# zhihu/rucene

Hardware: NVIDIA H100
Metric: queries/sec (higher is better)
Workload: dtype u32/f32

## Files before the change

### rucene_b200/csrc/gpu/eval_shared.cuh

```cuda
#pragma once
#include "engine.hpp"
#include "unpack.cuh"

namespace rg {

constexpr int kEvalThreads = 256;
constexpr int kEvalWarps = kEvalThreads / 32;
constexpr int kNewcMax = 512;
constexpr int kMaxK = 1024;
constexpr uint32_t kNone = 0xffffffffu;
constexpr uint32_t kRunMin = 256;
constexpr uint32_t kRunFirst = 63;
constexpr uint32_t kSent = 0x7fc0dead;
constexpr uint32_t kExcl = 0x7fc0beef;

struct EmitShared {
    float topk[kMaxK];
    float newc[kNewcMax];
    uint32_t warp_c[kEvalWarps], warp_m[kEvalWarps];
    uint32_t newc_n;
    uint32_t topk_n;
    float theta_local;
    uint32_t theta_in;
    uint32_t run_slot, run_cap, run_cnt;
// ... 207 lines not shown
        }
    }
    __syncthreads();
    if (nc && !es.overflow) {
        uint32_t pos = es.write_base + es.warp_c[warp];
        const uint32_t lt = (1u << lane) - 1u;
#pragma unroll
        for (int s = 0; s < STEPS; s++) {
            if ((cmask[s] >> lane) & 1u) {
                p.cand_arena[pos + __popc(cmask[s] & lt)] = rg_hit{doc[s] + doc_base, score[s]};
                const uint32_t i = atomicAdd(&es.newc_n, 1u);
                if (DEEP) deep_count(reinterpret_cast<uint32_t*>(es.topk), dmap, score[s]);
                else if (i < (uint32_t)kNewcMax) es.newc[i] = score[s];
            }
            pos += __popc(cmask[s]);
        }
    }
    __syncthreads();
    if (warp == 0) {
        if (DEEP) theta_update_deep(es, p, item_idx, dmap);
        else theta_update(es, p.k, p.item_theta + item_idx);
    }
}

__device__ __forceinline__ uint32_t lower_bound_i32(const int32_t* __restrict__ a, uint32_t lo,
                                                    uint32_t hi, int32_t key) {
    while (lo < hi) {
        const uint32_t mid = (lo + hi) >> 1;
        if (__ldg(a + mid) < key) lo = mid + 1;
        else hi = mid;
    }
    return lo;
}
__device__ __forceinline__ uint32_t lower_bound_gallop(const int32_t* __restrict__ a, uint32_t hint,
                                                       uint32_t n, int32_t key) {
    uint32_t lo = hint, step = 1, hi = hint;
    while (hi < n && __ldg(a + hi) < key) {
        lo = hi + 1;
        hi += step;
        step <<= 1;
    }
    return lower_bound_i32(a, lo, min(hi, n), key);
}

struct TermCtx {
    const int32_t* blk_last;
    const BlockDesc* blk_desc;
    const float* cache;
    uint32_t nb;
    uint32_t cur;
    uint32_t next_cur;
    uint32_t tail_n;
    uint32_t tail_pos;
    uint32_t tail_next;
    int32_t tail_base;
    float w1;
};

static __device__ void decode_tail(const SegDev& seg, const TermDev& td, int32_t* docs, int32_t* freqs) {
    if (td.doc_freq == 1) {
        docs[0] = td.singleton_doc;
        freqs[0] = td.singleton_freq;
        return;
    }
    const uint8_t* p = seg.tails + td.tail_off;
    uint32_t pos = 0;
    int32_t acc = td.tail_base;
    for (uint32_t i = 0; i < td.tail_n; i++) {
        const uint32_t code = (uint32_t)read_vint(p, pos);
        acc += (int32_t)(code >> 1);
        docs[i] = acc;
        freqs[i] = (code & 1u) ? 1 : read_vint(p, pos);
    }
}

__device__ __forceinline__ bool is_live(const SegDev& seg, int doc) {
    if (!seg.live) return true;
    return (seg.live[doc >> 6] >> (doc & 63)) & 1ull;
}

constexpr int kOrWarps = 1;
constexpr int kOrThreads = kOrWarps * 32;
constexpr int kWw = 768;
constexpr int kNewcW = 64;

struct WTerm {
    const int32_t* blk_last;
    union {
        const BlockDesc* blk_desc;
        const uint32_t* col_bmax;
    };
    union {
        const float* cache;
        const uint32_t* col_bits;
    };
    uint32_t nb;
    uint32_t cur;
    uint32_t n;
    uint32_t pos;
    uint32_t term_id;
    float w1;
    uint32_t is_not;
    uint32_t is_col;
    union {
        const uint4* pre;
        unsigned long long* col_dbg;
    };
};

struct MsmCtx {
    uint8_t* cnt;
    uint32_t msm;
    float* mx;
};
template <bool NOT, bool MSM, bool DMAX, bool POS = false>
__device__ __forceinline__ void accumulate_posting(uint32_t* acc, int idx, float s, bool is_not, bool live,
                                                   float te, uint32_t& hot, uint32_t& my_matches,
                                                   const MsmCtx& mc) {
    if (POS) {
        acc[idx] = __float_as_uint(__fadd_rn(__uint_as_float(acc[idx]), s));
        return;
    }
    const uint32_t old = acc[idx];
    if (!NOT || !is_not) {
        const float sum = __fadd_rn(old == kSent ? 0.0f : __uint_as_float(old), s);
        acc[idx] = __float_as_uint(sum);
        if (DMAX) mc.mx[idx] = old == kSent ? s : fmaxf(mc.mx[idx], s);
        if (MSM) {
            const uint32_t c = (uint32_t)mc.cnt[idx] + 1u;
            mc.cnt[idx] = (uint8_t)c;
            if (c == mc.msm && live) my_matches++;
        } else if (old == kSent && live) {
            my_matches++;
        }
        if (DMAX || sum > te) hot |= 1u << (idx >> 5);
    } else if (old != kSent && old != kExcl) {
        acc[idx] = kExcl;
        if (live && (!MSM || mc.cnt[idx] >= mc.msm)) my_matches--;
    }
}

struct alignas(16) WarpShared {
    uint32_t acc[kWw];
    WTerm term[kMaxTerms];
    float newc[kNewcW];
};

struct WEmit {
    float* topk;
    bool mirror;
    uint32_t topk_n;
    float theta_local;
    uint32_t theta_in;
    uint32_t run_slot, run_cap, run_cnt;
    uint32_t matches;
    bool overflow;
};

__device__ __forceinline__ void wtheta_recompute(const WEmit& em, uint32_t k, int lane, float& theta, int& argmin) {
    float m = INFINITY;
    int mi = 0;
    for (uint32_t j = lane; j < k; j += 32) {
        const float v = em.topk[j];
        if (v < m) {
            m = v;
            mi = (int)j;
        }
// ... 266 lines not shown
```

### rucene_b200/csrc/gpu/query_kernels.cu

```cuda
#include <algorithm>

#include "eval_shared.cuh"

namespace rg {


template <bool LIVE, bool EDGE, bool POS>
__device__ __forceinline__ void column_window(uint32_t* acc, const float* __restrict__ col, bool every_doc,
                                              const SegDev& seg, int win0, int wlen, int first_in, float te, int lane,
                                              uint32_t& hot, uint32_t& my_matches) {
    if (POS && !EDGE && wlen == kWw) {
#pragma unroll
        for (int h = 0; h < kWw / 128; h += 3) {
            float4 v[3];
#pragma unroll
            for (int j = 0; j < 3; j++) v[j] = __ldg(reinterpret_cast<const float4*>(col + win0 + lane * 4 + (h + j) * 128));
#pragma unroll
            for (int j = 0; j < 3; j++) {
                float4* a = reinterpret_cast<float4*>(acc + lane * 4 + (h + j) * 128);
                const float4 o = *a;
                *a = make_float4(__fadd_rn(o.x, v[j].x), __fadd_rn(o.y, v[j].y), __fadd_rn(o.z, v[j].z), __fadd_rn(o.w, v[j].w));
            }
        }
        return;
    }
#pragma unroll 2
    for (int i = lane * 4; i < wlen; i += 128) {
        const int d0 = win0 + i;
        const float4 v = __ldg(reinterpret_cast<const float4*>(col + d0));
        float sv[4] = {v.x, v.y, v.z, v.w};
        const uint4 o4 = *reinterpret_cast<const uint4*>(acc + i);
        uint32_t o[4] = {o4.x, o4.y, o4.z, o4.w};
        bool any_hot = false;
        if (POS) {
#pragma unroll
            for (int q = 0; q < 4; q++) {
                if (EDGE) sv[q] = (i + q >= first_in && i + q < wlen) ? sv[q] : 0.0f;
                o[q] = __float_as_uint(__fadd_rn(__uint_as_float(o[q]), sv[q]));
            }
        } else {
            uint32_t live4 = 0xfu;
            if (LIVE && seg.live) live4 = (uint32_t)(seg.live[d0 >> 6] >> (d0 & 63)) & 0xfu;
#pragma unroll
            for (int q = 0; q < 4; q++) {
                bool present = every_doc || sv[q] != 0.0f;
                if (EDGE) present = present && i + q >= first_in && i + q < wlen;
                const bool fresh = o[q] == kSent;
                const float sum = __fadd_rn(fresh ? 0.0f : __uint_as_float(o[q]), sv[q]);
                o[q] = present ? __float_as_uint(sum) : o[q];
                my_matches += (fresh && present && (!LIVE || ((live4 >> q) & 1u))) ? 1u : 0u;
                any_hot |= present && sum > te;
            }
        }
        *reinterpret_cast<uint4*>(acc + i) = make_uint4(o[0], o[1], o[2], o[3]);
        if (!POS) hot |= any_hot ? 1u << (i >> 5) : 0u;
    }
}

__device__ __forceinline__ uint32_t min1(uint32_t x) {
    uint32_t r;
    asm("min.u32 %0, %1, 1;" : "=r"(r) : "r"(x));
    return r;
}
template <bool LIVE>
__device__ __forceinline__ void count_and_max(const uint4 o, int g, int lane, const uint64_t* __restrict__ live, int win0,
                                              uint32_t& matches, float& mx) {
    if (LIVE && live) {
        uint32_t m4 = (o.x != 0u ? 1u : 0u) | (o.y != 0u ? 2u : 0u) | (o.z != 0u ? 4u : 0u) | (o.w != 0u ? 8u : 0u);
        if (m4) {
            const int d0 = win0 + (g * 32 + lane) * 4;
            uint32_t l4 = 0;
#pragma unroll
            for (int q = 0; q < 4; q++) l4 |= ((live[(d0 + q) >> 6] >> ((d0 + q) & 63)) & 1ull) ? 1u << q : 0u;
            m4 &= l4;
        }
        matches += __popc(m4);
    } else {
        matches += (min1(o.x) + min1(o.y)) + (min1(o.z) + min1(o.w));
    }
    mx = fmaxf(fmaxf(mx, __uint_as_float(o.x)), fmaxf(fmaxf(__uint_as_float(o.y), __uint_as_float(o.z)), __uint_as_float(o.w)));
}

template <bool LIVE, bool BOUND = false>
__device__ __noinline__ uint32_t columns_only_window(const WTerm* term, uint32_t active, const uint64_t* __restrict__ live,
                                                     int win0, int hi, float te, int lane) {
    uint32_t c = 0;
    float mx = 0.0f;
    const int win1 = win0 + kWw;
    if (BOUND) {
        const int b0 = win0 / kColBlk;
        uint32_t m = 0;
        bool ok = true;
        if ((active >> lane) & 1u) {
            const uint32_t* bm = term[lane].col_bmax;
            ok = bm != nullptr;
            if (ok) {
#pragma unroll
                for (int j = 0; j <= kWw / kColBlk; j++)
                    m = max(m, b0 + j <= (win1 - 1) / kColBlk ? __ldg(bm + b0 + j) : 0u);
            }
        }
        bool clear = false;
        if (__all_sync(0xffffffffu, ok)) {
            float c_ub = __uint_as_float(m);
#pragma unroll
            for (int o = 16; o; o >>= 1) c_ub = __fadd_ru(c_ub, __shfl_xor_sync(0xffffffffu, c_ub, o));
            clear = c_ub <= __fmul_rd(te, 0.99999237060546875f);
        }
        unsigned long long* dbg = term[__ffs(active) - 1].col_dbg;
        if (dbg && lane == 0) atomicAdd(dbg + 13, clear ? 1ull : 1ull << 32);
        if (clear) {
            if (lane < kWw / 32) {
                const int d0 = win0 + lane * 32;
                uint32_t w = 0;
                for (uint32_t a = active; a; a &= a - 1) w |= __ldg(term[__ffs(a) - 1].col_bits + (d0 >> 5));
                if (LIVE && live) w &= (uint32_t)(live[d0 >> 6] >> (d0 & 32));
                c = __popc(w);
            }
            return c;
        }
    }
#pragma unroll
    for (int h = 0; h < kWw / 128; h += 3) {
        float4 s3[3];
#pragma unroll
        for (int j = 0; j < 3; j++) s3[j] = make_float4(0.0f, 0.0f, 0.0f, 0.0f);
        for (uint32_t m = active; m; m &= m - 1) {
            const float* col = reinterpret_cast<const float*>(term[__ffs(m) - 1].blk_last) + win0 + lane * 4;
            float4 v[3];
#pragma unroll
            for (int j = 0; j < 3; j++) v[j] = __ldg(reinterpret_cast<const float4*>(col + (h + j) * 128));
            if (h == 0 && lane < kWw / 32 && win1 + lane * 32 < hi)
                asm volatile("prefetch.global.L2 [%0];" ::"l"(col - lane * 4 + kWw + lane * 32));
#pragma unroll
            for (int j = 0; j < 3; j++)
                s3[j] = make_float4(__fadd_rn(s3[j].x, v[j].x), __fadd_rn(s3[j].y, v[j].y), __fadd_rn(s3[j].z, v[j].z),
                                    __fadd_rn(s3[j].w, v[j].w));
        }
#pragma unroll
        for (int j = 0; j < 3; j++)
            count_and_max<LIVE>(make_uint4(__float_as_uint(s3[j].x), __float_as_uint(s3[j].y), __float_as_uint(s3[j].z),
                                           __float_as_uint(s3[j].w)),
                                h + j, lane, live, win0, c, mx);
    }
    return __any_sync(0xffffffffu, mx > te) ? 0xffffffffu : c;
}

__device__ __forceinline__ int list_window(uint32_t* acc, WTerm& tc, int win0, int win1, int hi, int lane) {
    const uint32_t* list = reinterpret_cast<const uint32_t*>(tc.pre);
    const uint32_t nb = tc.nb;
    uint32_t b = tc.cur, pos = tc.pos;
    int nx = kNoMoreDocs;
    while (b < nb) {
        const uint32_t* blk = list + (size_t)b * (2 * kBlock);
        if (pos == 0 && (int)__ldg(blk + kBlock - 1) < win1) {
            const uint4 dv = __ldg(reinterpret_cast<const uint4*>(blk) + lane);
            const uint4 sv = __ldg(reinterpret_cast<const uint4*>(blk) + 32 + lane);
            if (b + 1 < nb && lane < 8) asm volatile("prefetch.global.L2 [%0];" ::"l"(blk + 2 * kBlock + lane * 32));
            const uint32_t d[4] = {dv.x, dv.y, dv.z, dv.w}, s[4] = {sv.x, sv.y, sv.z, sv.w};
#pragma unroll
            for (int q = 0; q < 4; q++) {
                uint32_t* a = acc + ((int)d[q] - win0);
                *a = __float_as_uint(__fadd_rn(__uint_as_float(*a), __uint_as_float(s[q])));
            }
            b++;
            continue;
        }
        const uint32_t i = pos + lane;
        const int d = i < (uint32_t)kBlock ? (int)__ldg(blk + i) : kNoMoreDocs;
        const float s = i < (uint32_t)kBlock ? __uint_as_float(__ldg(blk + kBlock + i)) : 0.0f;
        const bool in_win = d < win1;
        const uint32_t c = __popc(__ballot_sync(0xffffffffu, in_win));
        if (in_win) acc[d - win0] = __float_as_uint(__fadd_rn(__uint_as_float(acc[d - win0]), s));
        pos += c;
        if (pos == (uint32_t)kBlock) {
            b++;
            pos = 0;
        } else if (c < 32) {
            nx = __shfl_sync(0xffffffffu, d, c);
            break;
        }
    }
    if (nx >= hi) b = nb;
    tc.cur = b;
    tc.pos = pos;
    return b < nb ? nx : kNoMoreDocs;
}

template <bool LIVE, bool NOT, bool MSM, bool DMAX, bool POS, bool LEAN = false, bool DEEP = false>
__global__ void __launch_bounds__(kOrThreads, LEAN ? 32 : 24)
k_eval_or(EvalParams p, const uint32_t* __restrict__ item_ids, uint32_t n_ids, uint32_t warp_bytes,
          uint32_t kcap) {
    static_assert(!LEAN || (POS && !NOT && !MSM && !DMAX), "the decode-free variant is plain-sum only");
    extern __shared__ __align__(16) unsigned char smem_raw[];
    const int lane = lane_id(), warp = threadIdx.x >> 5;
    const uint32_t wid = blockIdx.x * kOrWarps + warp;
    if (wid >= n_ids) return;
    unsigned char* base = smem_raw + (size_t)warp * warp_bytes;
    WarpShared& sh = *reinterpret_cast<WarpShared*>(base);
    float* topk = reinterpret_cast<float*>(base + sizeof(WarpShared));
    int32_t* cdocs = reinterpret_cast<int32_t*>(topk + kcap);
    const uint32_t item_idx = item_ids[wid];
    const WorkItem it = p.items[item_idx];
    const SegDev seg = p.segs[it.seg];
    const int T = it.n_terms;
    const int lo = it.lo, hi = it.hi;
    float* cscores = reinterpret_cast<float*>(cdocs + T * kBlock);
    const uint2 dmap = DEEP ? p.deep_map[it.query] : uint2{0u, 0u};

    for (int i = lane; i < kWw; i += 32) sh.acc[i] = POS ? 0u : kSent;
    MsmCtx mc;
    mc.cnt = reinterpret_cast<uint8_t*>(cscores + T * kBlock);
    mc.msm = max(1u, (uint32_t)it.type >> kItemMsmShift);
    mc.mx = reinterpret_cast<float*>(mc.cnt + kWw);
    const bool dmax_item = DMAX && (it.type & kItemDismax) != 0;
    const float tie = dmax_item ? p.clauses[it.clause_begin + T].weight : 0.0f;
    if (MSM) {
        for (int i = lane; i < kWw / 4; i += 32) reinterpret_cast<uint32_t*>(mc.cnt)[i] = 0u;
    }
    if (lane < T && (p.clauses[it.clause_begin + lane].flags & kClauseColumn)) {
        const ItemClause c = p.clauses[it.clause_begin + lane];
        WTerm& tc = sh.term[lane];
        tc.blk_last = reinterpret_cast<const int32_t*>(p.cols[c.term_id].col);
        tc.col_bmax = LEAN && p.cols[c.term_id].bits ? p.cols[c.term_id].bmax : nullptr;
        tc.col_bits = LEAN ? p.cols[c.term_id].bits : nullptr;
        tc.nb = 0;
        tc.cur = 1;
        tc.n = 0;
        tc.pos = 0;
        tc.term_id = c.term_id;
        tc.w1 = 0.0f;
        tc.is_not = 0;
        tc.is_col = (c.flags & kClauseAllDocs) ? 2 : 1;
        tc.col_dbg = LEAN ? p.dbg : nullptr;
    } else if (lane < T) {
        const ItemClause c = p.clauses[it.clause_begin + lane];
        const TermDev td = seg.terms[c.term_id];
        WTerm& tc = sh.term[lane];
        tc.is_col = 0;
        tc.pre = (c.flags & kClauseList) ? reinterpret_cast<const uint4*>(p.cols[c.flags >> kClauseRefShift].col) : nullptr;
        tc.blk_last = seg.blk_last + td.blk_begin;
        tc.blk_desc = seg.blk_desc + td.blk_begin;
        tc.cache = p.caches + (size_t)c.cache_id * 256;
        tc.nb = LEAN ? td.n_blocks + (td.tail_n ? 1u : 0u) : td.n_blocks;
        tc.cur = lower_bound_i32(tc.blk_last, 0, td.n_blocks, lo);
        tc.n = 0;
        tc.pos = 0;
        tc.term_id = c.term_id;
        tc.w1 = __fmul_rn(c.weight, __fadd_rn(p.k1, 1.0f));
        tc.is_not = c.flags & kClauseNot;
    }
    __syncwarp();
    const bool my_stream = lane < T && sh.term[lane < T ? lane : 0].is_col == 0;
    uint32_t hot = 0, my_matches = 0;
    int nd = kNoMoreDocs;
    for (int t = 0; t < T && LEAN; t++) {
        WTerm& tc = sh.term[t];
        if (tc.is_col || tc.cur >= tc.nb) continue;
        const uint32_t* blk = reinterpret_cast<const uint32_t*>(tc.pre) + (size_t)tc.cur * (2 * kBlock);
        const uint4 dv = __ldg(reinterpret_cast<const uint4*>(blk) + lane);
        const uint32_t pos = __reduce_add_sync(0xffffffffu, ((int)dv.x < lo) + ((int)dv.y < lo) + ((int)dv.z < lo) +
                                                                ((int)dv.w < lo));
        const int first = (int)__ldg(blk + pos);
        __syncwarp();
        tc.pos = pos;
        if (lane == t) nd = first < hi ? first : kNoMoreDocs;
    }
    for (int t = 0; t < T && !LEAN; t++) {
        if (stream_refill<LIVE, NOT, MSM, DMAX, POS>(seg, p, sh.term[t], cdocs + t * kBlock, cscores + t * kBlock, lo, hi,
                                                lane, 0, -2147483647 - 1, sh.acc, hot, my_matches, INFINITY, mc)) {
            const int first = cdocs[t * kBlock + sh.term[t].pos];
            if (lane == t) nd = first;
        }
    }
    if (lane < T && sh.term[lane].is_col && lo < hi) nd = lo & (LEAN ? ~31 : ~3);
    int w0 = __reduce_min_sync(0xffffffffu, nd);

    WEmit em;
    em.topk = topk;
    em.topk_n = 0;
    em.theta_local = -INFINITY;
    em.theta_in = 0;
    em.run_slot = kNone;
    em.run_cap = 0;
    em.run_cnt = 0;
    em.matches = 0;
    em.overflow = false;
    if (DEEP) em.theta_local = deep_inherit(reinterpret_cast<uint32_t*>(topk), p, item_idx, it.chain_pos, dmap, lane);
    else wtheta_inherit(em, p, item_idx, it.chain_pos, kcap, lane);
    const bool lb_ok = (uint32_t)lane < it.chain_pos;
    uint32_t win_no = 0;

    while (w0 < hi) {
        const int win0 = w0;
        const int win1 = hi - win0 > kWw ? win0 + kWw : hi;
        uint32_t inherited = 0;
        if ((win_no++ & 7u) == 0 && it.chain_pos) {
            inherited = lb_ok ? ld_volatile_u32(p.item_theta + item_idx - 1 - lane) : 0u;
            inherited = __reduce_max_sync(0xffffffffu, inherited);
        }
        hot = 0;
        if (inherited > em.theta_in) {
            em.theta_in = inherited;
            if (lane == 0) atomicMax(p.item_theta + item_idx, inherited);
        }
        float te = em.theta_local;
        if (em.theta_in > kOrderedNegInf) te = fmaxf(te, ordered_to_float(em.theta_in));
        const bool open = !POS && te == -INFINITY;
        if (POS) te = fmaxf(te, 0.0f);
        uint32_t active = __ballot_sync(0xffffffffu, nd < win1);
        if (POS && active && !__any_sync(0xffffffffu, my_stream && nd < win1) && win1 - win0 == kWw && win0 >= lo) {
            const uint32_t cnt = columns_only_window<LIVE, LEAN>(sh.term, active, seg.live, win0, hi, te, lane);
            if (cnt != 0xffffffffu) {
                my_matches += cnt;
                if ((active >> lane) & 1u) nd = win1 < hi ? win1 : kNoMoreDocs;
                const int next_doc = __reduce_min_sync(0xffffffffu, nd);
                if (next_doc == kNoMoreDocs) break;
                w0 = next_doc;
                continue;
            }
        }
        while (active) {
            const int t = __ffs(active) - 1;
            active &= active - 1;
            WTerm& tc = sh.term[t];
            if (tc.is_col) {
                const float* col = reinterpret_cast<const float*>(tc.blk_last);
                const int wlen = win1 - win0;
                if (lane < kWw / 32 && win1 + lane * 32 < hi)
                    asm volatile("prefetch.global.L2 [%0];" ::"l"(col + win1 + lane * 32));
                const int first_in = lo - win0;
                const bool every_doc = tc.is_col == 2;
                if (MSM || DMAX) {
                    for (int i = lane * 4; i < wlen; i += 128) {
                        const int d0 = win0 + i;
                        const float4 v = __ldg(reinterpret_cast<const float4*>(col + d0));
                        const float sv[4] = {v.x, v.y, v.z, v.w};
#pragma unroll
                        for (int q = 0; q < 4; q++) {
                            const int d = d0 + q;
                            if ((every_doc || sv[q] != 0.0f) && d >= lo && d < win1)
                                accumulate_posting<NOT, MSM, DMAX>(sh.acc, i + q, sv[q], false,
                                                                   LIVE ? is_live(seg, d) : true, te, hot, my_matches, mc);
                        }
                    }
                } else if (first_in > 0 || (wlen & 3)) {
                    column_window<LIVE, true, POS>(sh.acc, col, every_doc, seg, win0, wlen, first_in, te, lane, hot, my_matches);
                } else {
                    column_window<LIVE, false, POS>(sh.acc, col, every_doc, seg, win0, wlen, first_in, te, lane, hot, my_matches);
                }
                if (lane == t) nd = win1 < hi ? win1 : kNoMoreDocs;
                __syncwarp();
                continue;
            }
            if (LEAN) {
                const int nx = list_window(sh.acc, tc, win0, win1, hi, lane);
                if (lane == t) nd = nx;
                __syncwarp();
                continue;
            }
            const int32_t* cd = cdocs + t * kBlock;
            const float* cs = cscores + t * kBlock;
            uint32_t pos = tc.pos, n = tc.n;
            for (;;) {
                if (pos >= n) {
                    if (tc.cur > tc.nb) break;
                    __syncwarp();
                    if (!stream_refill<LIVE, NOT, MSM, DMAX, POS>(seg, p, tc, cdocs + t * kBlock, cscores + t * kBlock, lo, hi,
                                                             lane, win0, win1, sh.acc, hot, my_matches, te, mc)) {
                        pos = n = 0;
                        break;
                    }
                    pos = tc.pos;
                    n = tc.n;
                }
                const uint32_t i = pos + lane;
                const int d = i < n ? cd[i] : kNoMoreDocs;
                const float sv = i < n ? cs[i] : 0.0f;
                const bool in_win = d < win1;
                const uint32_t c = __popc(__ballot_sync(0xffffffffu, in_win));
                if (in_win)
                    accumulate_posting<NOT, MSM, DMAX, POS>(sh.acc, d - win0, sv, NOT && tc.is_not != 0,
                                                            (LIVE && !POS) ? is_live(seg, d) : true, te, hot, my_matches, mc);
                pos += c;
                if (c < 32 && pos < n) break;
            }
            tc.pos = pos;
            tc.n = n;
            const int nx = pos < n ? cd[pos] : kNoMoreDocs;
            if (lane == t) nd = nx;
            __syncwarp();
        }
        const int next_doc = __reduce_min_sync(0xffffffffu, nd);
        if (POS) {
            hot = 0;
            float mx = 0.0f;
#pragma unroll
            for (int g = 0; g < kWw / 128; g++)
                count_and_max<LIVE>(reinterpret_cast<const uint4*>(sh.acc)[g * 32 + lane], g, lane, seg.live, win0, my_matches, mx);
            if (__any_sync(0xffffffffu, mx > te)) {
#pragma unroll
                for (int g = 0; g < kWw / 128; g++) {
                    const float4 o = reinterpret_cast<const float4*>(sh.acc)[g * 32 + lane];
                    hot |= fmaxf(fmaxf(o.x, o.y), fmaxf(o.z, o.w)) > te ? 1u << (g * 4 + (lane >> 3)) : 0u;
                }
            }
        }
        hot = __reduce_or_sync(0xffffffffu, hot);
        {
            uint32_t newc_n = 0;
            while (hot) {
                const int s = __ffs(hot) - 1;
                hot &= hot - 1;
                const int idx = s * 32 + lane;
                const uint32_t v = sh.acc[idx];
                float sc = __uint_as_float(v);
                if (DMAX && dmax_item) {
                    const float m = mc.mx[idx];
                    sc = __fadd_rn(m, __fmul_rn(__fsub_rn(sc, m), tie));
                }
                const bool cand = POS ? (sc > te && (LIVE ? is_live(seg, win0 + idx) : true))
                                      : (v != kSent && (!NOT || v != kExcl) && (open || sc > te) &&
                                         (!MSM || mc.cnt[idx] >= mc.msm) && (LIVE ? is_live(seg, win0 + idx) : true));
                const uint32_t cm = __ballot_sync(0xffffffffu, cand);
                if (!cm || em.overflow) continue;
                const uint32_t c = __popc(cm);
                CandRun* hdr = reinterpret_cast<CandRun*>(p.cand_arena);
                if (em.run_slot == kNone || em.run_cnt + c > em.run_cap) {
                    uint32_t slot = 0;
                    const uint32_t cap = em.run_slot == kNone ? kRunFirst : kRunMin;
                    if (lane == 0) {
                        const unsigned long long s64 = atomicAdd(p.arena_next, (unsigned long long)cap + 1ull);
                        slot = (s64 + cap + 1ull > (unsigned long long)p.arena_slots) ? kNone : (uint32_t)s64;
                        if (slot == kNone) atomicOr(p.error_flag, 1u);
                        else if (em.run_slot == kNone) p.item_head[item_idx] = slot;
                        else hdr[em.run_slot] = CandRun{slot, em.run_cnt};
                    }
                    slot = __shfl_sync(0xffffffffu, slot, 0);
                    if (slot == kNone) {
                        em.overflow = true;
                        continue;
                    }
                    em.run_slot = slot;
                    em.run_cap = cap;
                    em.run_cnt = 0;
                }
                if (cand) {
                    const uint32_t r = __popc(cm & ((1u << lane) - 1u));
                    p.cand_arena[em.run_slot + 1 + em.run_cnt + r] = rg_hit{win0 + idx + seg.doc_base, sc};
                    if (DEEP) deep_count(reinterpret_cast<uint32_t*>(topk), dmap, sc);
                    else if (newc_n + r < (uint32_t)kNewcW) sh.newc[newc_n + r] = sc;
                }
                em.run_cnt += c;
                newc_n += c;
                if (lane == 0) hdr[em.run_slot] = CandRun{kNone, em.run_cnt};
            }
            __syncwarp();
#pragma unroll
            for (int g = 0; g < kWw / 128; g++) {
                const uint32_t z = POS ? 0u : kSent;
                reinterpret_cast<uint4*>(sh.acc)[g * 32 + lane] = make_uint4(z, z, z, z);
            }
            if (MSM) {
                for (int i = lane; i < kWw / 16; i += 32) reinterpret_cast<uint4*>(mc.cnt)[i] = make_uint4(0, 0, 0, 0);
            }
            if (DEEP) wtheta_update_deep(em, p, item_idx, dmap, lane, newc_n);
            else wtheta_update(em, p, item_idx, kcap, lane, sh.newc, newc_n);
            __syncwarp();
        }
        if (next_doc == kNoMoreDocs) break;
        w0 = next_doc;
    }
    my_matches = __reduce_add_sync(0xffffffffu, my_matches);
    if (lane == 0) p.item_matches[item_idx] = my_matches;
}

constexpr int kAndSlots = kEvalWarps * kBlock;
constexpr int kAndSteps = kBlock / 32;

struct AndShared {
    int32_t ldoc[kAndSlots];
    float lscore[kAndSlots];
    int32_t slab_docs[kEvalWarps][kBlock];
    int32_t slab_freqs[kEvalWarps][kBlock];
    TermCtx term[kMaxTerms];
    uint32_t term_id[kMaxTerms];
    uint32_t is_not[kMaxTerms];
    uint32_t is_opt[kMaxTerms];
    const float* colp[kMaxTerms];
    uint32_t hint[kEvalWarps][kMaxTerms];
    float oscore[kAndSlots];
    uint32_t mmask[kEvalWarps][kAndSteps];
    EmitShared emit;
};

constexpr uint32_t kOptScoreThreshold = 100;

struct AndSharedR : AndShared {
    RangeRef rref[kMaxTerms];
    uint32_t is_rng[kMaxTerms];
    int32_t rblk[kEvalWarps];
    uint32_t rcur;
};

struct AndSharedN : AndSharedR {
    int32_t gdoc[kEvalWarps][kBlock];
    float gscore[kEvalWarps][kBlock];
    float gsum[kAndSlots];
    int32_t gpos[kEvalWarps];
    int32_t gend[kEvalWarps];
    int32_t gn[kEvalWarps];
    uint32_t gblk[kEvalWarps];
    uint32_t gdone[kEvalWarps];
    uint32_t grp[kMaxTerms];
    int32_t gx;
};

__device__ __forceinline__ bool range_hit(const RangeRef& r, int d) {
    const uint32_t o0 = __ldg(r.offsets + d), o1 = __ldg(r.offsets + d + 1);
    for (uint32_t j = o0; j < o1; j++) {
        const uint64_t key = r.wide ? __ldg(static_cast<const unsigned long long*>(r.keys) + j)
                                    : (uint64_t)__ldg(static_cast<const uint32_t*>(r.keys) + j);
        if (key > r.upper) return false;
        if (key >= r.lower) return true;
    }
    return false;
}

template <bool REQOPT, bool OTHER, bool RANGES, bool GROUPS = false, bool DEEP = false>
__device__ __forceinline__ void eval_and_body(const EvalParams& p, const uint32_t* __restrict__ item_ids,
                                              const RangeParams& rp, unsigned long long* gstats = nullptr) {
    extern __shared__ __align__(16) unsigned char smem_raw[];
    AndShared& sh = *reinterpret_cast<AndShared*>(smem_raw);
    AndSharedR& shr = *reinterpret_cast<AndSharedR*>(smem_raw);
    AndSharedN& shn = *reinterpret_cast<AndSharedN*>(smem_raw);
    const uint32_t item_idx = item_ids[blockIdx.x];
    const WorkItem it = p.items[item_idx];
    const SegDev seg = p.segs[it.seg];
    const int lane = lane_id(), warp = threadIdx.x >> 5;
    const int T = it.n_terms;
    const int lo = it.lo, hi = it.hi;

    emit_init(sh.emit);
    if ((int)threadIdx.x < T) {
        const ItemClause c = p.clauses[it.clause_begin + threadIdx.x];
        const bool is_col = (c.flags & kClauseColumn) != 0;
        const bool is_rng = RANGES && (c.flags & kClauseRange) != 0;
        if (RANGES) {
            shr.is_rng[threadIdx.x] = is_rng;
            if (is_rng) shr.rref[threadIdx.x] = rp.ranges[c.term_id];
        }
        if (GROUPS) shn.grp[threadIdx.x] = c.flags & (kClauseReqGroup | kClauseOptGroup | kClauseGroupLast);
        const TermDev td = (is_col || is_rng) ? TermDev{} : seg.terms[c.term_id];
        TermCtx& tc = sh.term[threadIdx.x];
        sh.term_id[threadIdx.x] = c.term_id;
        sh.is_not[threadIdx.x] = c.flags & kClauseNot;
        sh.is_opt[threadIdx.x] = (c.flags / kClauseOpt) & 1u;
// ... 762 lines not shown
        return;
    }
    const float* cache = caches + (size_t)job.cache_id * 256;
    if (MODE == 2 || MODE == 3) {
        uint32_t* bits = static_cast<uint32_t*>(job.dst);
        const float tau1 = job.weight, tau2 = __uint_as_float(job.pad);
#pragma unroll
        for (int q = 0; q < 4; q++) {
            if (d[q] < 0 || d[q] >= seg.max_doc) continue;
            const float nrm = seg.norms ? __ldg(cache + __ldg(seg.norms + d[q])) : k1;
            const float fq = (float)f[q];
            const float t = __fdiv_ru(fq, __fadd_rd(fq, nrm));
            if (MODE == 3) {
                const int bin = t > 0.0f ? min(255, (int)ceilf(t * 256.0f) - 1) : 0;
                atomicAdd(hist + (size_t)jl * 256 + (t <= 1.0f ? bin : 255), 1u);
            } else {
                if (!(t <= tau1)) atomicOr(bits + (d[q] >> 5), 1u << (d[q] & 31));
                if (!(t <= tau2)) atomicOr(bits + plane_stride + (d[q] >> 5), 1u << (d[q] & 31));
            }
        }
        return;
    }
    float* col = static_cast<float*>(job.dst);
    const float w1 = __fmul_rn(job.weight, __fadd_rn(k1, 1.0f));
    if (MODE == 4) {
        uint32_t dv[4], sv[4];
#pragma unroll
        for (int q = 0; q < 4; q++) {
            const bool ok = d[q] >= 0 && d[q] < seg.max_doc;
            const float nrm = seg.norms ? __ldg(cache + __ldg(seg.norms + (ok ? d[q] : 0))) : k1;
            dv[q] = ok ? (uint32_t)d[q] : (uint32_t)kNoMoreDocs;
            sv[q] = ok ? __float_as_uint(bm25_score(w1, (float)f[q], nrm)) : 0u;
        }
        uint4* blk = static_cast<uint4*>(job.dst) + (size_t)b * 64;
        blk[lane] = make_uint4(dv[0], dv[1], dv[2], dv[3]);
        blk[32 + lane] = make_uint4(sv[0], sv[1], sv[2], sv[3]);
        return;
    }
#pragma unroll
    for (int q = 0; q < 4; q++) {
        if (d[q] < 0 || d[q] >= seg.max_doc) continue;
        const float nrm = seg.norms ? __ldg(cache + __ldg(seg.norms + d[q])) : k1;
        col[d[q]] = bm25_score(w1, (float)f[q], nrm);
    }
}

void launch_build_columns(cudaStream_t st, const SegDev* segs, const ColumnJob* jobs, uint32_t n_jobs,
                          uint32_t n_units, const float* caches, float k1) {
    if (!n_jobs || !n_units) return;
    k_build_columns<0><<<(n_units + kColWarps - 1) / kColWarps, kColWarps * 32, 0, st>>>(segs, jobs, n_jobs, n_units,
                                                                                         caches, k1, nullptr, 0);
}
__global__ void __launch_bounds__(256) k_col_block_max(const float* __restrict__ col, uint32_t* __restrict__ bmax, uint32_t n_blk) {
    static_assert(kColBlk == 128, "one float4 per lane");
    const uint32_t b = blockIdx.x * 8 + (threadIdx.x >> 5);
    if (b >= n_blk) return;
    const uint4 v = __ldg(reinterpret_cast<const uint4*>(col + (size_t)b * kColBlk) + lane_id());
    const uint32_t m = __reduce_max_sync(0xffffffffu, max(max(v.x, v.y), max(v.z, v.w)));
    if (lane_id() == 0) bmax[b] = m;
}
void launch_col_block_max(cudaStream_t st, const float* col, uint32_t* bmax, uint32_t n_blk) {
    if (!n_blk) return;
    k_col_block_max<<<(n_blk + 7) / 8, 256, 0, st>>>(col, bmax, n_blk);
}
void launch_build_lists(cudaStream_t st, const SegDev* segs, const ColumnJob* jobs, uint32_t n_jobs, uint32_t n_units,
                        const float* caches, float k1) {
    if (!n_jobs || !n_units) return;
    k_build_columns<4><<<(n_units + kColWarps - 1) / kColWarps, kColWarps * 32, 0, st>>>(segs, jobs, n_jobs, n_units,
                                                                                         caches, k1, nullptr, 0);
}
void launch_build_bitmaps(cudaStream_t st, const SegDev* seg, const ColumnJob* jobs, uint32_t n_jobs,
                          uint32_t n_units) {
    if (!n_jobs || !n_units) return;
    k_build_columns<1><<<(n_units + kColWarps - 1) / kColWarps, kColWarps * 32, 0, st>>>(seg, jobs, n_jobs, n_units,
                                                                                         nullptr, 0.f, nullptr, 0);
}
void launch_build_tf_planes(cudaStream_t st, const SegDev* segs, const ColumnJob* jobs, uint32_t n_jobs,
                            uint32_t n_units, const float* caches, float k1, uint32_t* hist, size_t plane_stride) {
    if (!n_jobs || !n_units) return;
    const uint32_t ctas = (n_units + kColWarps - 1) / kColWarps;
    if (hist) k_build_columns<3><<<ctas, kColWarps * 32, 0, st>>>(segs, jobs, n_jobs, n_units, caches, k1, hist, 0);
    else k_build_columns<2><<<ctas, kColWarps * 32, 0, st>>>(segs, jobs, n_jobs, n_units, caches, k1, nullptr, plane_stride);
}
template <bool LIVE, bool NOT, bool MSM, bool DMAX, bool POS = false, bool LEAN = false, bool DEEP = false>
static void launch_eval_or_t(cudaStream_t st, const EvalParams& p, const uint32_t* item_ids, uint32_t n, size_t wb,
                             uint32_t kcap) {
    const size_t smem = wb * kOrWarps;
    cudaFuncSetAttribute(k_eval_or<LIVE, NOT, MSM, DMAX, POS, LEAN, DEEP>, cudaFuncAttributeMaxDynamicSharedMemorySize, (int)smem);
    const uint32_t ctas = (n + kOrWarps - 1) / kOrWarps;
    k_eval_or<LIVE, NOT, MSM, DMAX, POS, LEAN, DEEP><<<ctas, kOrThreads, smem, st>>>(p, item_ids, n, (uint32_t)wb, kcap);
}
void launch_eval_or_lean(cudaStream_t st, const EvalParams& p, const uint32_t* item_ids, uint32_t n, bool has_live) {
    if (!n) return;
    const bool deep = p.k > (uint32_t)kMaxK;
    const uint32_t kcap = deep ? (uint32_t)kDeepBuckets : (std::min<uint32_t>(p.k, kMaxK) + 31u) & ~31u;
    const size_t wb = (sizeof(WarpShared) + (size_t)kcap * sizeof(float) + 15) & ~size_t(15);
    if (deep && has_live) launch_eval_or_t<true, false, false, false, true, true, true>(st, p, item_ids, n, wb, kcap);
    else if (deep) launch_eval_or_t<false, false, false, false, true, true, true>(st, p, item_ids, n, wb, kcap);
    else if (has_live) launch_eval_or_t<true, false, false, false, true, true>(st, p, item_ids, n, wb, kcap);
    else launch_eval_or_t<false, false, false, false, true, true>(st, p, item_ids, n, wb, kcap);
}
template <bool DEEP>
static void launch_eval_or_d(cudaStream_t st, const EvalParams& p, const uint32_t* item_ids, uint32_t n,
                             uint32_t max_terms, bool has_live, bool has_not, bool has_msm, bool has_dmax, bool all_pos);
void launch_eval_or(cudaStream_t st, const EvalParams& p, const uint32_t* item_ids, uint32_t n,
                    uint32_t max_terms, bool has_live, bool has_not, bool has_msm, bool has_dmax, bool all_pos) {
    if (!n) return;
    if (p.k > (uint32_t)kMaxK) launch_eval_or_d<true>(st, p, item_ids, n, max_terms, has_live, has_not, has_msm, has_dmax, all_pos);
    else launch_eval_or_d<false>(st, p, item_ids, n, max_terms, has_live, has_not, has_msm, has_dmax, all_pos);
}
template <bool DEEP>
static void launch_eval_or_d(cudaStream_t st, const EvalParams& p, const uint32_t* item_ids, uint32_t n,
                             uint32_t max_terms, bool has_live, bool has_not, bool has_msm, bool has_dmax, bool all_pos) {
    const uint32_t kcap = DEEP ? (uint32_t)kDeepBuckets : (std::min<uint32_t>(p.k, kMaxK) + 31u) & ~31u;
    size_t wb = sizeof(WarpShared) + (size_t)kcap * sizeof(float) + (size_t)max_terms * kBlock * 8;
    wb = (wb + 15) & ~size_t(15);
    if (has_dmax) {
        wb += kWw + kWw * sizeof(float);
        wb = (wb + 15) & ~size_t(15);
        launch_eval_or_t<true, true, true, true, false, false, DEEP>(st, p, item_ids, n, wb, kcap);
    } else if (has_msm) {
        wb += kWw;
        wb = (wb + 15) & ~size_t(15);
        launch_eval_or_t<true, true, true, false, false, false, DEEP>(st, p, item_ids, n, wb, kcap);
    } else if (has_live && has_not) launch_eval_or_t<true, true, false, false, false, false, DEEP>(st, p, item_ids, n, wb, kcap);
    else if (has_not) launch_eval_or_t<false, true, false, false, false, false, DEEP>(st, p, item_ids, n, wb, kcap);
    else if (has_live && all_pos) launch_eval_or_t<true, false, false, false, true, false, DEEP>(st, p, item_ids, n, wb, kcap);
    else if (all_pos) launch_eval_or_t<false, false, false, false, true, false, DEEP>(st, p, item_ids, n, wb, kcap);
    else if (has_live) launch_eval_or_t<true, false, false, false, false, false, DEEP>(st, p, item_ids, n, wb, kcap);
    else launch_eval_or_t<false, false, false, false, false, false, DEEP>(st, p, item_ids, n, wb, kcap);
}
template <bool REQOPT, bool OTHER, bool DEEP>
static void launch_eval_and_t(cudaStream_t st, const EvalParams& p, const uint32_t* item_ids, uint32_t n) {
    cudaFuncSetAttribute(k_eval_and<REQOPT, OTHER, DEEP>, cudaFuncAttributeMaxDynamicSharedMemorySize,
                         (int)sizeof(AndShared));
    k_eval_and<REQOPT, OTHER, DEEP><<<n, kEvalThreads, sizeof(AndShared), st>>>(p, item_ids);
}
template <bool DEEP>
static void launch_eval_and_d(cudaStream_t st, const EvalParams& p, const uint32_t* item_ids, uint32_t n, bool req_opt,
                              bool has_other_enc) {
    if (req_opt && has_other_enc) launch_eval_and_t<true, true, DEEP>(st, p, item_ids, n);
    else if (req_opt) launch_eval_and_t<true, false, DEEP>(st, p, item_ids, n);
    else if (has_other_enc) launch_eval_and_t<false, true, DEEP>(st, p, item_ids, n);
    else launch_eval_and_t<false, false, DEEP>(st, p, item_ids, n);
}
void launch_eval_and(cudaStream_t st, const EvalParams& p, const uint32_t* item_ids, uint32_t n, bool req_opt,
                     bool has_other_enc) {
    if (!n) return;
    if (p.k > (uint32_t)kMaxK) launch_eval_and_d<true>(st, p, item_ids, n, req_opt, has_other_enc);
    else launch_eval_and_d<false>(st, p, item_ids, n, req_opt, has_other_enc);
}
template <bool REQOPT, bool OTHER, bool DEEP>
static void launch_eval_and_ranges_t(cudaStream_t st, const EvalParams& p, const RangeParams& rp,
                                     const uint32_t* item_ids, uint32_t n) {
    cudaFuncSetAttribute(k_eval_and_ranges<REQOPT, OTHER, DEEP>, cudaFuncAttributeMaxDynamicSharedMemorySize,
                         (int)sizeof(AndSharedR));
    k_eval_and_ranges<REQOPT, OTHER, DEEP><<<n, kEvalThreads, sizeof(AndSharedR), st>>>(p, item_ids, rp);
}
template <bool DEEP>
static void launch_eval_and_ranges_d(cudaStream_t st, const EvalParams& p, const RangeParams& rp,
                                     const uint32_t* item_ids, uint32_t n, bool req_opt, bool has_other_enc) {
    if (req_opt && has_other_enc) launch_eval_and_ranges_t<true, true, DEEP>(st, p, rp, item_ids, n);
    else if (req_opt) launch_eval_and_ranges_t<true, false, DEEP>(st, p, rp, item_ids, n);
    else if (has_other_enc) launch_eval_and_ranges_t<false, true, DEEP>(st, p, rp, item_ids, n);
    else launch_eval_and_ranges_t<false, false, DEEP>(st, p, rp, item_ids, n);
}
void launch_eval_and_ranges(cudaStream_t st, const EvalParams& p, const RangeParams& rp, const uint32_t* item_ids,
                            uint32_t n, bool req_opt, bool has_other_enc) {
    if (!n) return;
    if (p.k > (uint32_t)kMaxK) launch_eval_and_ranges_d<true>(st, p, rp, item_ids, n, req_opt, has_other_enc);
    else launch_eval_and_ranges_d<false>(st, p, rp, item_ids, n, req_opt, has_other_enc);
}
template <bool REQOPT, bool OTHER, bool DEEP>
static void launch_eval_and_nested_t(cudaStream_t st, const EvalParams& p, const RangeParams& rp,
                                     unsigned long long* gstats, const uint32_t* item_ids, uint32_t n) {
    cudaFuncSetAttribute(k_eval_and_nested<REQOPT, OTHER, DEEP>, cudaFuncAttributeMaxDynamicSharedMemorySize,
                         (int)sizeof(AndSharedN));
    k_eval_and_nested<REQOPT, OTHER, DEEP><<<n, kEvalThreads, sizeof(AndSharedN), st>>>(p, item_ids, rp, gstats);
}
template <bool DEEP>
static void launch_eval_and_nested_d(cudaStream_t st, const EvalParams& p, const RangeParams& rp,
                                     unsigned long long* gstats, const uint32_t* item_ids, uint32_t n, bool req_opt,
                                     bool has_other_enc) {
// ... 40 lines not shown
```

Measured before the change: 12410.

## Stream column loads past L1, shrink newc window, add lean-kernel stats

```diff
diff --git a/rucene_b200/csrc/gpu/eval_shared.cuh b/rucene_b200/csrc/gpu/eval_shared.cuh
--- a/rucene_b200/csrc/gpu/eval_shared.cuh
+++ b/rucene_b200/csrc/gpu/eval_shared.cuh
@@ -313,7 +313,7 @@
 constexpr int kOrWarps = 1;
 constexpr int kOrThreads = kOrWarps * 32;
 constexpr int kWw = 768;
-constexpr int kNewcW = 64;
+constexpr int kNewcW = 16;
 
 struct WTerm {
     const int32_t* blk_last;
diff --git a/rucene_b200/csrc/gpu/query_kernels.cu b/rucene_b200/csrc/gpu/query_kernels.cu
--- a/rucene_b200/csrc/gpu/query_kernels.cu
+++ b/rucene_b200/csrc/gpu/query_kernels.cu
@@ -4,6 +4,12 @@
 
 namespace rg {
 
+
+__device__ __forceinline__ float4 ld_col4(const float* p) {
+    float4 v;
+    asm("ld.global.nc.L1::no_allocate.v4.f32 {%0, %1, %2, %3}, [%4];" : "=f"(v.x), "=f"(v.y), "=f"(v.z), "=f"(v.w) : "l"(p));
+    return v;
+}
 
 template <bool LIVE, bool EDGE, bool POS>
 __device__ __forceinline__ void column_window(uint32_t* acc, const float* __restrict__ col, bool every_doc,
@@ -14,7 +20,7 @@
         for (int h = 0; h < kWw / 128; h += 3) {
             float4 v[3];
 #pragma unroll
-            for (int j = 0; j < 3; j++) v[j] = __ldg(reinterpret_cast<const float4*>(col + win0 + lane * 4 + (h + j) * 128));
+            for (int j = 0; j < 3; j++) v[j] = ld_col4(col + win0 + lane * 4 + (h + j) * 128);
 #pragma unroll
             for (int j = 0; j < 3; j++) {
                 float4* a = reinterpret_cast<float4*>(acc + lane * 4 + (h + j) * 128);
@@ -27,7 +33,7 @@
 #pragma unroll 2
     for (int i = lane * 4; i < wlen; i += 128) {
         const int d0 = win0 + i;
-        const float4 v = __ldg(reinterpret_cast<const float4*>(col + d0));
+        const float4 v = ld_col4(col + d0);
         float sv[4] = {v.x, v.y, v.z, v.w};
         const uint4 o4 = *reinterpret_cast<const uint4*>(acc + i);
         uint32_t o[4] = {o4.x, o4.y, o4.z, o4.w};
@@ -129,7 +135,7 @@
             const float* col = reinterpret_cast<const float*>(term[__ffs(m) - 1].blk_last) + win0 + lane * 4;
             float4 v[3];
 #pragma unroll
-            for (int j = 0; j < 3; j++) v[j] = __ldg(reinterpret_cast<const float4*>(col + (h + j) * 128));
+            for (int j = 0; j < 3; j++) v[j] = ld_col4(col + (h + j) * 128);
             if (h == 0 && lane < kWw / 32 && win1 + lane * 32 < hi)
                 asm volatile("prefetch.global.L2 [%0];" ::"l"(col - lane * 4 + kWw + lane * 32));
 #pragma unroll
@@ -146,10 +152,17 @@
     return __any_sync(0xffffffffu, mx > te) ? 0xffffffffu : c;
 }
 
-__device__ __forceinline__ int list_window(uint32_t* acc, WTerm& tc, int win0, int win1, int hi, int lane) {
+constexpr int kStWindows = 0;
+constexpr int kStListActs = 1;
+constexpr int kStListPostings = 2;
+constexpr int kStScanned = 3;
+constexpr int kLeanStats = 4;
+
+__device__ __forceinline__ int list_window(uint32_t* acc, WTerm& tc, int win0, int win1, int hi, int lane, uint32_t* st) {
     const uint32_t* list = reinterpret_cast<const uint32_t*>(tc.pre);
     const uint32_t nb = tc.nb;
     uint32_t b = tc.cur, pos = tc.pos;
+    if (st && lane == 0) st[kStListPostings] -= b * kBlock + pos;
     int nx = kNoMoreDocs;
     while (b < nb) {
         const uint32_t* blk = list + (size_t)b * (2 * kBlock);
@@ -181,17 +194,22 @@
             break;
         }
     }
+    if (st && lane == 0) {
+        st[kStListActs]++;
+        st[kStListPostings] += b * kBlock + pos;
+    }
     if (nx >= hi) b = nb;
     tc.cur = b;
     tc.pos = pos;
     return b < nb ? nx : kNoMoreDocs;
 }
 
-template <bool LIVE, bool NOT, bool MSM, bool DMAX, bool POS, bool LEAN = false, bool DEEP = false>
+template <bool LIVE, bool NOT, bool MSM, bool DMAX, bool POS, bool LEAN = false, bool DEEP = false, bool STATS = false>
 __global__ void __launch_bounds__(kOrThreads, LEAN ? 32 : 24)
 k_eval_or(EvalParams p, const uint32_t* __restrict__ item_ids, uint32_t n_ids, uint32_t warp_bytes,
           uint32_t kcap) {
     static_assert(!LEAN || (POS && !NOT && !MSM && !DMAX), "the decode-free variant is plain-sum only");
+    static_assert(!STATS || LEAN, "only the decode-free variant counts events");
     extern __shared__ __align__(16) unsigned char smem_raw[];
     const int lane = lane_id(), warp = threadIdx.x >> 5;
     const uint32_t wid = blockIdx.x * kOrWarps + warp;
@@ -207,6 +225,8 @@
     const int lo = it.lo, hi = it.hi;
     float* cscores = reinterpret_cast<float*>(cdocs + T * kBlock);
     const uint2 dmap = DEEP ? p.deep_map[it.query] : uint2{0u, 0u};
+    uint32_t* const st = STATS ? reinterpret_cast<uint32_t*>(cdocs) : nullptr;
+    if (STATS && lane < kLeanStats) st[lane] = 0u;
 
     for (int i = lane; i < kWw; i += 32) sh.acc[i] = POS ? 0u : kSent;
     MsmCtx mc;
@@ -300,6 +320,7 @@
             inherited = __reduce_max_sync(0xffffffffu, inherited);
         }
         hot = 0;
+        if (STATS && lane == 0) st[kStWindows]++;
         if (inherited > em.theta_in) {
             em.theta_in = inherited;
             if (lane == 0) atomicMax(p.item_theta + item_idx, inherited);
@@ -354,7 +375,7 @@
                 continue;
             }
             if (LEAN) {
-                const int nx = list_window(sh.acc, tc, win0, win1, hi, lane);
+                const int nx = list_window(sh.acc, tc, win0, win1, hi, lane, st);
                 if (lane == t) nd = nx;
                 __syncwarp();
                 continue;
@@ -407,6 +428,7 @@
             }
         }
         hot = __reduce_or_sync(0xffffffffu, hot);
+        if (STATS && lane == 0 && hot) st[kStScanned]++;
         {
             uint32_t newc_n = 0;
             while (hot) {
@@ -473,6 +495,11 @@
     }
     my_matches = __reduce_add_sync(0xffffffffu, my_matches);
     if (lane == 0) p.item_matches[item_idx] = my_matches;
+    if (STATS && lane == 0) {
+        const int slot[kLeanStats] = {1, 7, 5, 11};
+#pragma unroll
+        for (int i = 0; i < kLeanStats; i++) atomicAdd(p.dbg + slot[i], (unsigned long long)st[i]);
+    }
 }
 
 constexpr int kAndSlots = kEvalWarps * kBlock;
@@ -1401,23 +1428,30 @@
     if (hist) k_build_columns<3><<<ctas, kColWarps * 32, 0, st>>>(segs, jobs, n_jobs, n_units, caches, k1, hist, 0);
     else k_build_columns<2><<<ctas, kColWarps * 32, 0, st>>>(segs, jobs, n_jobs, n_units, caches, k1, nullptr, plane_stride);
 }
-template <bool LIVE, bool NOT, bool MSM, bool DMAX, bool POS = false, bool LEAN = false, bool DEEP = false>
+template <bool LIVE, bool NOT, bool MSM, bool DMAX, bool POS = false, bool LEAN = false, bool DEEP = false, bool STATS = false>
 static void launch_eval_or_t(cudaStream_t st, const EvalParams& p, const uint32_t* item_ids, uint32_t n, size_t wb,
                              uint32_t kcap) {
     const size_t smem = wb * kOrWarps;
-    cudaFuncSetAttribute(k_eval_or<LIVE, NOT, MSM, DMAX, POS, LEAN, DEEP>, cudaFuncAttributeMaxDynamicSharedMemorySize, (int)smem);
+    cudaFuncSetAttribute(k_eval_or<LIVE, NOT, MSM, DMAX, POS, LEAN, DEEP, STATS>, cudaFuncAttributeMaxDynamicSharedMemorySize,
+                         (int)smem);
     const uint32_t ctas = (n + kOrWarps - 1) / kOrWarps;
-    k_eval_or<LIVE, NOT, MSM, DMAX, POS, LEAN, DEEP><<<ctas, kOrThreads, smem, st>>>(p, item_ids, n, (uint32_t)wb, kcap);
+    k_eval_or<LIVE, NOT, MSM, DMAX, POS, LEAN, DEEP, STATS><<<ctas, kOrThreads, smem, st>>>(p, item_ids, n, (uint32_t)wb, kcap);
+}
+template <bool STATS>
+static void launch_eval_or_lean_t(cudaStream_t st, const EvalParams& p, const uint32_t* item_ids, uint32_t n, bool has_live) {
+    const bool deep = p.k > (uint32_t)kMaxK;
+    const uint32_t kcap = deep ? (uint32_t)kDeepBuckets : (std::min<uint32_t>(p.k, kMaxK) + 31u) & ~31u;
+    const size_t wb = (sizeof(WarpShared) + (size_t)kcap * sizeof(float) + (STATS ? kLeanStats * sizeof(uint32_t) : 0) + 15) &
+                      ~size_t(15);
+    if (deep && has_live) launch_eval_or_t<true, false, false, false, true, true, true, STATS>(st, p, item_ids, n, wb, kcap);
+    else if (deep) launch_eval_or_t<false, false, false, false, true, true, true, STATS>(st, p, item_ids, n, wb, kcap);
+    else if (has_live) launch_eval_or_t<true, false, false, false, true, true, false, STATS>(st, p, item_ids, n, wb, kcap);
+    else launch_eval_or_t<false, false, false, false, true, true, false, STATS>(st, p, item_ids, n, wb, kcap);
 }
 void launch_eval_or_lean(cudaStream_t st, const EvalParams& p, const uint32_t* item_ids, uint32_t n, bool has_live) {
     if (!n) return;
-    const bool deep = p.k > (uint32_t)kMaxK;
-    const uint32_t kcap = deep ? (uint32_t)kDeepBuckets : (std::min<uint32_t>(p.k, kMaxK) + 31u) & ~31u;
-    const size_t wb = (sizeof(WarpShared) + (size_t)kcap * sizeof(float) + 15) & ~size_t(15);
-    if (deep && has_live) launch_eval_or_t<true, false, false, false, true, true, true>(st, p, item_ids, n, wb, kcap);
-    else if (deep) launch_eval_or_t<false, false, false, false, true, true, true>(st, p, item_ids, n, wb, kcap);
-    else if (has_live) launch_eval_or_t<true, false, false, false, true, true>(st, p, item_ids, n, wb, kcap);
-    else launch_eval_or_t<false, false, false, false, true, true>(st, p, item_ids, n, wb, kcap);
+    if (p.dbg) launch_eval_or_lean_t<true>(st, p, item_ids, n, has_live);
+    else launch_eval_or_lean_t<false>(st, p, item_ids, n, has_live);
 }
 template <bool DEEP>
 static void launch_eval_or_d(cudaStream_t st, const EvalParams& p, const uint32_t* item_ids, uint32_t n,
```

Result: faster. 12780, median of 6 (+3.0%).
